# Chyaboiii/antidote_ccrdt

Hardware: AMD Instinct MI355X
Metric: CRDT ops/sec (topk_rmv, 1M keys, 8-DC vclocks) (higher is better)
Workload: dtype int64

## Files before the change

antidote_ccrdt_amd/csrc/engine.cpp:

```cpp
#include <algorithm>
#include <chrono>
#include <cstdio>
#include <cstdlib>
#include <cstring>
#include <mutex>
#include <numeric>
#include <string>
#include <thread>
#include <tuple>
#include <vector>

#include "common.hpp"
#include "engine.hpp"
#include "trmv_kernels.hpp"

namespace ccrdt {

static thread_local std::string g_last_error;
void set_error(const std::string& msg) { g_last_error = msg; }

int trmv_launch_scan(const TrmvApplyArgs& a, uint64_t* partials, uint32_t* key_rmv, hipStream_t st);
void trmv_kernels_preload();
void trmv_wave_preload();
void trmv_resident_preload();
void trmv_steady_preload();
int trmv_launch_validate(const TrmvApplyArgs& a, uint64_t n_ops, uint32_t* err, unsigned long long* scratch,
                         hipStream_t st);
int trmv_launch_mark_done(uint8_t* done, uint64_t n_keys, const uint32_t* list, uint32_t n_list, const uint32_t* n_dev,
                          uint32_t* ex_cnt, hipStream_t st);
int trmv_launch_keep(const TrmvApplyArgs& a, uint32_t grid, hipStream_t st);
int trmv_launch_downstream(const TrmvDownArgs& a, hipStream_t st);
int trmv_launch_wave(const TrmvApplyArgs& a, uint64_t grid_keys, hipStream_t st);
int trmv_launch_first_list(const uint64_t* key_ptr, uint64_t n_keys, uint32_t thresh, uint32_t* list,
                           uint32_t* count, hipStream_t st);
uint32_t trmv_wave_waves(uint64_t grid_keys);
int trmv_launch_resident_consume(const TrmvApplyArgs& a, uint32_t waves, hipStream_t st);
int trmv_launch_steady(const TrmvApplyArgs& a, int cls, uint64_t grid_keys, hipStream_t st);
int trmv_launch_resident(const TrmvApplyArgs& a, uint64_t grid_keys, hipStream_t st);
int trmv_launch_steady_hbm(const TrmvApplyArgs& a, uint32_t waves, void* scratch, hipStream_t st);
uint64_t trmv_steady_hbm_bytes(bool ranked);
uint32_t trmv_steady_hbm_players();
int trmv_launch_replica_vc(const int64_t* vc, uint64_t n_keys, int n_dc, int64_t* out,
                           hipStream_t st);
int trmv_launch_pack_extras(const uint64_t* key_ptr, const uint32_t* ex_cnt, const TrmvExtraRec* ex,
                            const int64_t* ex_vc, uint64_t n_keys, int n_dc, int64_t* rows,
                            int64_t cap, uint32_t* count, hipStream_t st);
int trmv_launch_exchange_pack(const int64_t* vc, const uint64_t* key_ptr, const uint32_t* ex_cnt,
                              const TrmvExtraRec* ex, const int64_t* ex_vc, uint64_t n_keys, int n_dc, int64_t* pack,
                              int64_t cap, const int64_t* op_map, int64_t n_map, uint32_t host_word, hipStream_t st);
int trmv_launch_exchange_reduce(const int64_t* g, int world, int64_t len, int n_dc, int64_t* hdr, int64_t* out,
                                hipStream_t st);

static constexpr int TRMV_N_TIERS = 5;
static constexpr int TRMV_TIER_LAST = 4;
static constexpr uint32_t TRMV_HBM_WAVES = 128;
static constexpr int TRMV_STATUS_WORDS = 2 + 2 * TRMV_N_TIERS;
static constexpr uint32_t TRMV_LATER_GRID = 4096;

template <class F>
void for_key_ranges_host(uint64_t n, F f) {
  const unsigned hw = std::thread::hardware_concurrency();
  uint64_t nt = std::min<uint64_t>(16, hw ? hw : 1);
  nt = std::min<uint64_t>(nt, n / 4096 + 1);
  std::vector<std::thread> pool;
  for (uint64_t t = 1; t < nt; ++t) pool.emplace_back([&, t] { f(n * t / nt, n * (t + 1) / nt); });
  f(0, n / nt);
  for (auto& th : pool) th.join();
}
// ... 319 lines not shown
        used += c - E.arena_sub[0][i][x];
        room += E.arena_sub[1][i][x] - c;
      }
      const uint64_t take = used - std::min(used, E.arena_used[x]);
      E.arena_used[x] = used;
      E.arena_rate[x] = std::max(E.arena_rate[x], take);
      roomy &= room >= 2 * take;
    }
    E.inplace_ready = roomy;
    const uint32_t* lc = reinterpret_cast<const uint32_t*>(static_cast<const char*>(E.h_arena) + 2 * ARENA_RB);
    for (int l = 0; l < 3; ++l) {
      uint32_t n = 0;
      for (int i = 0; i < TRMV_NSUB; ++i) n += lc[4 * i + l];
      E.trmv_overflow_keys[6 + l] = n;
    }
  }
  float mv = 0.f, mr = 0.f;
  CCRDT_HIP(hipEventElapsedTime(&mv, E.evt[0], E.evt[1]));
  CCRDT_HIP(hipEventElapsedTime(&mr, E.evt[1], E.evt[2]));
  E.trmv_tier_ms[5] += mv;
  E.trmv_tier_ms[3] += mr;
  handed = hs[2 + 2 * 3];
  E.trmv_overflow_keys[5] = handed;
  (void)D;
  return CCRDT_OK;
}

int trmv_pass_full(Engine& E, TrmvApplyArgs a, uint64_t n_ops, uint32_t* status, int& first_tier, int& n_over) {
  const int D = E.n_dc;
  const uint64_t nk = (uint64_t)E.n_keys;
  const int out = 1 - E.cur, mout = 1 - E.mcur;
  a.inplace = 0;
  a.fresh = E.fresh ? 1 : 0;
  if (a.key_done) {
    const char* ff = getenv("CCRDT_TRMV_FAIL_FINISH");
    if (ff && ff[0] == '1') {
      set_error("trmv_apply: injected failure of the finishing pass (CCRDT_TRMV_FAIL_FINISH)");
      return CCRDT_ENOMEM;
    }
  }
  a.slack = E.k <= 128 ? trmv_pool_slack() : 0;
  if (E.fresh && !E.fresh_room) a.slack = 0;
  if (E.fresh && a.slack)
    for (int x = 0; x < 3; ++x)
      if (trmv_fresh_off(true, x, nk, n_ops) >= 0xFFFFFFFFull) a.slack = 0;
  a.old_s = E.trmv_side(E.mcur, E.cur);
  CCRDT_TRY(E.trmv[mout].meta.ensure(nk * sizeof(KeyMeta)));
  CCRDT_TRY(E.trmv[mout].cap.ensure(nk * sizeof(KeyCap)));
  a.new_s = E.trmv_side(mout, out);
  const uint64_t nb = (nk + 1023) / 1024;
  CCRDT_TRY(E.partials.ensure((nb * 3 + 3) * sizeof(uint64_t) + nk * sizeof(uint32_t)));
  uint64_t tot[3];
  for (int x = 0; x < 3; ++x) tot[x] = trmv_fresh_off(a.slack != 0, x, nk, n_ops);
  if (!E.fresh && nk) {
    CCRDT_TRY(trmv_launch_scan(a, E.partials.as<uint64_t>(),
                               reinterpret_cast<uint32_t*>(E.partials.as<uint64_t>() + nb * 3 + 3), E.stream));
    CCRDT_HIP(hipMemcpyAsync(E.h_status, E.partials.as<uint64_t>() + nb * 3, 3 * sizeof(uint64_t),
                             hipMemcpyDeviceToHost, E.stream));
    CCRDT_HIP(hipStreamSynchronize(E.stream));
    memcpy(tot, E.h_status, sizeof(tot));
  }
  if (tot[0] >= 0xFFFFFFFFull || tot[1] >= 0xFFFFFFFFull || tot[2] >= 0xFFFFFFFFull) {
    set_error("trmv_apply: resident state would exceed 2^32 elements");
    return CCRDT_ENOMEM;
  }
  auto grow = [&](TrmvBufs& b, bool room) -> int {
// ... 40 lines not shown
  auto segment = [&](int c0, int c1) -> int {
    const int e0 = ev;
    CCRDT_HIP(hipEventRecord(E.evt[ev++], E.stream));
    for (int ci = c0; ci < c1 && nk; ++ci) {
      const int t = chain[ci];
      DevBuf* ovf = &E.tier_ovf[t];
      a.key_list = work ? work->as<uint32_t>() : nullptr;
      a.n_list = work ? 0u : (uint32_t)nk;
      a.n_list_dev = n_dev;
      a.ovf_list = ovf->as<uint32_t>();
      a.status = status + 2 + 2 * t;
      const uint64_t grid = work ? later_grid : nk;
      if (t == 0) CCRDT_TRY(trmv_launch_wave(a, grid, E.stream));
      else if (t == 3) CCRDT_TRY(trmv_launch_resident(a, grid, E.stream));
      else CCRDT_TRY(trmv_launch_steady(a, t - 1, grid, E.stream));
      CCRDT_HIP(hipEventRecord(E.evt[ev++], E.stream));
      work = ovf;
      n_dev = a.status;
    }
    CCRDT_HIP(hipMemcpyAsync(E.h_status, status, TRMV_STATUS_WORDS * 4, hipMemcpyDeviceToHost, E.stream));
    CCRDT_HIP(hipStreamSynchronize(E.stream));
    uint32_t err = 0;
    for (int ci = c0; ci < c1; ++ci) err |= hs[3 + 2 * chain[ci]];
    if (err) return trmv_err_code(err);
    for (int ci = c0; ci < c1 && nk; ++ci) {
      const int t = chain[ci];
      float ms = 0.f;
      CCRDT_HIP(hipEventElapsedTime(&ms, E.evt[e0 + ci - c0], E.evt[e0 + ci - c0 + 1]));
      E.trmv_tier_ms[t] += ms;
      E.trmv_overflow_keys[t] = hs[2 + 2 * t];
    }
    return CCRDT_OK;
  };
  static const bool overlap_env = [] {
    const char* v = getenv("CCRDT_TRMV_OVERLAP");
    return !(v && v[0] == '0');
  }();
  static const uint64_t overlap_keys = [] {
    const char* v = getenv("CCRDT_TRMV_OVERLAP_KEYS");
    return v ? strtoull(v, nullptr, 10) : (1ull << 18);
  }();
  static const uint32_t overlap_waves = [] {
    const char* v = getenv("CCRDT_TRMV_OVERLAP_WAVES");
    const int x = v ? atoi(v) : 32;
    return (uint32_t)(x < 1 ? 1 : (x > 4096 ? 4096 : x));
  }();
  auto head_overlapped = [&]() -> int {
    if (!E.stream2) {
      int lo = 0, hi = 0;
      CCRDT_HIP(hipDeviceGetStreamPriorityRange(&lo, &hi));
      CCRDT_HIP(hipStreamCreateWithPriority(&E.stream2, hipStreamNonBlocking, hi));
      CCRDT_HIP(hipEventCreateWithFlags(&E.ev_ovl, hipEventDisableTiming));
    }
    constexpr uint32_t O_CLAIM = TRMV_NDONE, O_NFIRST = TRMV_NDONE + 1, O_PUB = TRMV_NDONE + 4;
    CCRDT_TRY(E.first_list.ensure(nk * 4));
    CCRDT_TRY(E.ovl.ensure((O_PUB + nk) * 4));
    uint32_t* ov = E.ovl.as<uint32_t>();
    CCRDT_HIP(hipMemsetAsync(ov, 0, (O_PUB + nk) * 4, E.stream));
    const uint32_t pmax = (uint32_t)std::min<int64_t>(E.k, 128);
    const uint32_t thresh = std::min<uint32_t>(128u, pmax + pmax / 5);
    CCRDT_TRY(trmv_launch_first_list(a.key_ptr, nk, thresh, E.first_list.as<uint32_t>(), ov + O_NFIRST, E.stream));
    const int e0 = ev;
    CCRDT_HIP(hipEventRecord(E.evt[ev++], E.stream));
    TrmvApplyArgs a0 = a;
    a0.key_list = nullptr;
    a0.n_list = (uint32_t)nk;
    a0.n_list_dev = nullptr;
    a0.ovf_list = E.tier_ovf[0].as<uint32_t>();
    a0.status = status + 2;
    a0.first_list = E.first_list.as<uint32_t>();
    a0.n_first = ov + O_NFIRST;
    a0.first_thresh = thresh;
    a0.pub = ov + O_PUB;
    a0.n_pub = (uint32_t)nk;
    a0.done = ov;
    CCRDT_TRY(trmv_launch_wave(a0, nk, E.stream));
    CCRDT_HIP(hipEventRecord(E.evt[ev++], E.stream));
    CCRDT_HIP(hipStreamWaitEvent(E.stream2, E.evt[e0], 0));
    TrmvApplyArgs a3 = a;
    a3.key_list = E.tier_ovf[0].as<uint32_t>();
    a3.n_list = 0;
    a3.n_list_dev = status + 2;
    a3.ovf_list = E.tier_ovf[3].as<uint32_t>();
    a3.status = status + 2 + 2 * 3;
    a3.pub = ov + O_PUB;
    a3.n_pub = (uint32_t)nk;
    a3.done = ov;
    a3.prod_waves = trmv_wave_waves(nk);
    a3.claim = ov + O_CLAIM;
    const char* stall_env = getenv("CCRDT_TRMV_OVERLAP_STALL");
    const bool force_stall = stall_env && stall_env[0] == '1';
    a3.spin_limit = force_stall ? 0u : (1u << 19);
    CCRDT_TRY(trmv_launch_resident_consume(a3, overlap_waves, E.stream2));
    CCRDT_HIP(hipEventRecord(E.ev_ovl, E.stream2));
    CCRDT_HIP(hipStreamWaitEvent(E.stream, E.ev_ovl, 0));
    CCRDT_HIP(hipEventRecord(E.evt[ev++], E.stream));
    CCRDT_HIP(hipMemcpyAsync(E.h_status, status, TRMV_STATUS_WORDS * 4, hipMemcpyDeviceToHost, E.stream));
    CCRDT_HIP(hipStreamSynchronize(E.stream));
    if ((hs[3 + 2 * 3] & TRMV_ERR_STALL) || force_stall) {
      CCRDT_HIP(hipMemsetAsync(status + 2 + 2 * 3, 0, 8, E.stream));
      a3.pub = nullptr;
      a3.done = nullptr;
      CCRDT_TRY(trmv_launch_resident(a3, later_grid, E.stream));
      CCRDT_HIP(hipEventRecord(E.evt[ev - 1], E.stream));
      CCRDT_HIP(hipMemcpyAsync(E.h_status, status, TRMV_STATUS_WORDS * 4, hipMemcpyDeviceToHost, E.stream));
      CCRDT_HIP(hipStreamSynchronize(E.stream));
      E.trmv_overflow_keys[9] = 1;
    }
    const uint32_t err = hs[3] | hs[3 + 2 * 3];
    if (err) return trmv_err_code(err);
    float m0 = 0.f, m3 = 0.f;
    CCRDT_HIP(hipEventElapsedTime(&m0, E.evt[e0], E.evt[e0 + 1]));
    CCRDT_HIP(hipEventElapsedTime(&m3, E.evt[e0 + 1], E.evt[e0 + 2]));
    E.trmv_tier_ms[0] += m0;
    E.trmv_tier_ms[3] += m3;
    E.trmv_overflow_keys[0] = hs[2];
    E.trmv_overflow_keys[3] = hs[2 + 2 * 3];
    work = &E.tier_ovf[3];
    n_dev = status + 2 + 2 * 3;
    return CCRDT_OK;
  };
// ... 946 lines not shown
```

antidote_ccrdt_amd/csrc/trmv_kernels.hpp:

```cpp
#pragma once
#include <cstdint>

namespace ccrdt {

constexpr uint32_t NONE16 = 0xFFFFu;
constexpr uint32_t NONE32 = 0xFFFFFFFFu;
constexpr int TRMV_DPAD = 8;
constexpr uint32_t TRMV_SEG_MAX = 0xFFFFu;

struct alignas(32) KeyMeta {
  uint32_t p_off, m_off, r_off;
  uint32_t np;
  uint32_t nm;
  uint32_t nr;
  uint32_t nobs;
  uint32_t minq;
};
static_assert(sizeof(KeyMeta) == 32, "KeyMeta is one 32-byte record");

struct alignas(16) KeyCap {
  uint32_t p_cap, m_cap, r_cap;
  uint16_t m_top;
  uint16_t flags;
};
// ... 37 lines not shown
  const uint8_t* dc;
  const int64_t* ts;
  const int64_t* rmv_vc;
  int64_t n_rmv_rows;
  TrmvSide old_s;
  TrmvSide new_s;
  int32_t fresh;
  uint32_t* ex_cnt;
  TrmvExtraRec* ex;
  int64_t* ex_vc;
  const uint32_t* key_list;
  uint32_t n_list;
  const uint32_t* n_list_dev;
  uint32_t* ovf_list;
  uint32_t* status;
  uint8_t* op_pl;
  int32_t inplace;
  unsigned long long* arena;
  const unsigned long long* arena_lim;
  uint32_t* lay_cnt;
  uint16_t* obs_ord;
  const uint8_t* key_done;
  const uint32_t* verr;
  int32_t slack;
  const uint32_t* first_list;
  const uint32_t* n_first;
  uint32_t first_thresh;
  uint32_t n_pub;
  uint32_t prod_waves;
  uint32_t spin_limit;
  uint32_t* pub;
  uint32_t* done;
  uint32_t* claim;
};
constexpr int TRMV_NDONE = 64;
constexpr uint32_t TRMV_ERR_STALL = 1u << 30;

__device__ __forceinline__ uint32_t trmv_key_nops(const TrmvApplyArgs& a, uint64_t k, uint64_t op0) {
  return (a.key_done && a.key_done[k]) ? 0u : (uint32_t)(a.key_ptr[k + 1] - op0);
}

__device__ __forceinline__ const __attribute__((address_space(4))) TrmvApplyArgs* trmv_kargs() {
  return kernarg_as<TrmvApplyArgs>();
}

__host__ __device__ __forceinline__ uint64_t trmv_fresh_off(bool room, int x, uint64_t k, uint64_t o) {
  return room ? (x == 0 ? 3 * o + 16 * k : (x == 1 ? 6 * o + 32 * k : o + 8 * k)) : o;
}
__host__ __device__ __forceinline__ uint32_t trmv_fresh_cap(bool room, int x, uint32_t nops) {
  return room ? (x == 0 ? 3 * nops + 16 : (x == 1 ? 6 * nops + 32 : nops + 8)) : nops;
}

__device__ __forceinline__ KeyMeta trmv_new_meta(const TrmvApplyArgs& a, uint64_t k) {
  if (a.fresh) {
    KeyMeta m;
    const uint64_t o = a.key_ptr[k];
    m.p_off = (uint32_t)trmv_fresh_off(a.slack != 0, 0, k, o);
    m.m_off = (uint32_t)trmv_fresh_off(a.slack != 0, 1, k, o);
    m.r_off = (uint32_t)trmv_fresh_off(a.slack != 0, 2, k, o);
    m.np = m.nm = m.nr = m.nobs = 0;
    m.minq = NONE32;
    return m;
  }
  return a.new_s.meta[k];
}

// ... 26 lines not shown
```

antidote_ccrdt_amd/csrc/trmv_wave.hip:

```cpp
#include "common.hpp"
#include "trmv_kernels.hpp"

#ifdef TRMV_PROF
__device__ unsigned long long g_trmv_prof[16];
#define PROF_STAMP(v)                                                        \
  do {                                                                       \
    __builtin_amdgcn_sched_barrier(0);                                       \
    asm volatile("s_memtime %0\n\ts_waitcnt lgkmcnt(0)" : "=s"(v)::"memory"); \
    __builtin_amdgcn_sched_barrier(0);                                       \
  } while (0)
#define PROF_MARK(i)                                                         \
  do {                                                                       \
    unsigned long long _t;                                                   \
    PROF_STAMP(_t);                                                          \
    if (lane_id() == 0 && (key & 63u) == 3) atomicAdd(&g_trmv_prof[i], _t - prof_t);             \
    prof_t = _t;                                                             \
  } while (0)
#else
#define PROF_STAMP(v) (void)0
#define PROF_MARK(i) (void)0
#endif

namespace ccrdt {

namespace {
constexpr int W_HCAP = 256;
constexpr int W_ECAP = 128;
constexpr int W_PCAP = 128;
constexpr int W_RCAP = 24;
constexpr int W_WAVES = 1;
#define ST_OUT(p, v) (*(p) = (v))
#define LD_IN(p) (*(p))
constexpr int W_KPW = 8;
constexpr int W_MD = (W_KPW + 7) / 8;
static_assert(W_KPW >= 1 && W_KPW <= 64, "1..64 keys per wave chunk");
constexpr unsigned long long W_EMPTY = 0x8000000000000000ull;
constexpr uint32_t NONE8 = 0xFFu;
constexpr uint32_t HSINK = W_HCAP, ESINK = W_ECAP, PSINK = W_PCAP;

template <bool FRESH>
struct alignas(16) WaveLds {
  static constexpr int NS_ = FRESH ? 0 : 1;
  unsigned long long htab[W_HCAP + 2];
  int64_t esc[W_ECAP + 2];
  int64_t ets[W_ECAP + 2];
  int64_t rows[W_RCAP][TRMV_DPAD];
  unsigned long long vc[TRMV_DPAD + 2];
  uint32_t pcnt2[W_PCAP / 2 + 4];
  uint32_t rsrc[W_RCAP];
  uint16_t ekd[W_ECAP + 8];
  uint8_t hp[W_HCAP];
  uint8_t sorted[W_ECAP + 8];
  uint8_t slab[W_ECAP];
  uint8_t fin[NS_ * (W_ECAP + 8)];
  uint32_t pa[W_PCAP + 8];
  uint32_t pb[W_PCAP + 8];
  uint8_t pmoff[NS_ * (W_PCAP + 8)];
  uint8_t peb[NS_ * (W_PCAP + 8)];
  uint8_t cpl[W_PCAP + 8];
  uint8_t rl[W_RCAP + 8];
  uint32_t nex;
  __device__ __forceinline__ uint8_t& fa(uint32_t p, int b) { return reinterpret_cast<uint8_t*>(pa)[4 * p + b]; }
  __device__ __forceinline__ uint8_t& fb(uint32_t p, int b) { return reinterpret_cast<uint8_t*>(pb)[4 * p + b]; }
};
#define PSTART(p) L.fa((p), 0)
#define PLR(p) L.fa((p), 1)
#define PFLAG(p) L.fa((p), 2)
#define PCNTF(p) L.fa((p), 3)
#define POBS(p) L.fb((p), 0)
#define PROW(p) L.fb((p), 1)
#define PGB(p) L.fb((p), 2)
#define PSLOT(p) L.fb((p), 3)

#define KA trmv_kargs()

__device__ __forceinline__ uint32_t whash(int64_t id) {
  const uint64_t x = (uint64_t)id * 0x9E3779B97F4A7C15ull;
  return (uint32_t)(x >> 56);
}

template <class W>
__device__ __forceinline__ uint32_t pcnt_of(const W& L, uint32_t p) {
  return (L.pcnt2[p >> 1] >> (16 * (p & 1))) & 0xFFFFu;
}

template <class W>
__device__ __forceinline__ void wave_emit(const TrmvApplyArgs& a, W& L, uint64_t op0,
                                          uint64_t op, uint8_t kind, int64_t id, int64_t sc,
                                          uint32_t dc, int64_t ts, uint32_t row) {
  const uint32_t pos = atomicAdd(&L.nex, 1u);
  TrmvExtraRec r;
  r.op = (uint32_t)op;
  r.kind = kind;
  r.dc = (uint8_t)dc;
  r.pad = 0;
  r.id = id;
  r.score = sc;
  r.ts = ts;
  KA->ex[op0 + pos] = r;
  if (kind == CCRDT_TRMV_RMV)
    for (int d = 0; d < KA->n_dc; ++d) KA->ex_vc[(op0 + pos) * KA->n_dc + d] = L.rows[row][d];
}

struct KeyIn {
  uint64_t op0;
  uint32_t nops;
  KeyMeta nmeta;
  int64_t id[2], sc[2], ts[2];
  uint32_t kind[2], dc[2];
  int64_t rv[W_RCAP / 8];
};

struct ChunkHdr {
  uint32_t key;
  uint64_t lo, hi;
  uint32_t meta[W_MD];
  uint64_t skip;
};

__device__ __forceinline__ uint32_t wave_list_key(uint32_t i, uint32_t n_first) {
  if (KA->first_list) return i < n_first ? KA->first_list[i] : i - n_first;
  return KA->key_list ? KA->key_list[i] : i;
}

__device__ __forceinline__ void wave_load_chunk(const TrmvApplyArgs& a, uint32_t c0, uint32_t n,
                                                uint32_t n_first, ChunkHdr& h) {
  const int lane = lane_id();
  const uint32_t j = (uint32_t)lane < n ? (uint32_t)lane : 0u;
  h.key = wave_list_key(c0 + j, n_first);
  h.lo = KA->key_ptr[h.key];
  h.hi = KA->key_ptr[h.key + 1];
  h.skip = KA->first_list ? ballot((uint32_t)lane < n && c0 + j >= n_first && h.hi - h.lo > KA->first_thresh) : 0ull;
#pragma unroll
  for (int i = 0; i < W_MD; ++i) {
    const uint32_t m = 8 * i + (lane >> 3);
    const uint32_t jm = m < n ? m : 0u;
    const uint32_t km = shfl32(h.key, (int)jm);
    if (KA->fresh) {
      const uint32_t d = lane & 7;
      h.meta[i] = d < 3 ? (uint32_t)trmv_fresh_off(KA->slack != 0, (int)d, km, KA->key_ptr[km])
                        : (d == 7 ? NONE32 : 0u);
    } else {
      h.meta[i] = reinterpret_cast<const uint32_t*>(a.new_s.meta + km)[lane & 7];
    }
  }
}

__device__ __forceinline__ void wave_load_key(const TrmvApplyArgs& a, const ChunkHdr& h, uint32_t j,
                                              KeyIn& in) {
  const int lane = lane_id();
  in.op0 = (uint64_t)rl64((int64_t)h.lo, (int)j);
  in.nops = (uint32_t)((uint64_t)rl64((int64_t)h.hi, (int)j) - in.op0);
  uint32_t* m = reinterpret_cast<uint32_t*>(&in.nmeta);
#pragma unroll
  for (int d = 0; d < 8; ++d) {
    uint32_t v = 0;
#pragma unroll
    for (int i = 0; i < W_MD; ++i)
      if ((j >> 3) == (uint32_t)i) v = rl32(h.meta[i], (int)(8 * (j & 7) + d));
    m[d] = v;
  }
  const int64_t* idp = KA->id + in.op0;
  const int64_t* scp = KA->score + in.op0;
  const int64_t* tsp = KA->ts + in.op0;
  const uint8_t* kp = KA->kind + in.op0;
  const uint8_t* dp = KA->dc + in.op0;
#pragma unroll
  for (int s = 0; s < 2; ++s) {
    const uint32_t l = s * 64 + lane;
    const bool v = l < in.nops;
    in.id[s] = v ? LD_IN(idp + l) : 0;
    in.sc[s] = v ? LD_IN(scp + l) : 0;
    in.ts[s] = v ? LD_IN(tsp + l) : 0;
    in.kind[s] = v ? (uint32_t)LD_IN(kp + l) : 0u;
    in.dc[s] = v ? (uint32_t)LD_IN(dp + l) : 0u;
  }
}

template <class W>
__device__ __forceinline__ void wave_load_rows(const TrmvApplyArgs& a, W& L, KeyIn& in) {
  const int lane = lane_id();
#pragma unroll
  for (int s = 0; s < W_RCAP / 8; ++s) in.rv[s] = 0;
  bool r[2];
#pragma unroll
  for (int s = 0; s < 2; ++s)
    r[s] = (uint32_t)(s * 64 + lane) < in.nops && (in.kind[s] == 2 || in.kind[s] == 3);
  const uint64_t b0 = ballot(r[0]), b1 = ballot(r[1]);
  const uint32_t n0 = (uint32_t)__builtin_popcountll(b0);
  const uint32_t n = n0 + (uint32_t)__builtin_popcountll(b1);
  if (n == 0 || KA->n_rmv_rows <= 0) return;
#pragma unroll
  for (int s = 0; s < 2; ++s) {
    const uint32_t k = s ? n0 + mbcnt(b1) : mbcnt(b0);
    if (r[s] && k < (uint32_t)W_RCAP)
      L.rsrc[k] = (in.ts[s] >= 0 && in.ts[s] < KA->n_rmv_rows) ? (uint32_t)in.ts[s] : 0u;
  }
  wave_lds_sync();
  const uint32_t d = (lane & 7) < KA->n_dc ? (lane & 7) : 0u;
#pragma unroll
  for (int s = 0; s < W_RCAP / 8; ++s) {
    const uint32_t k = s * 8 + (lane >> 3);
    const uint32_t row = k < n ? L.rsrc[k] : 0u;
    in.rv[s] = KA->rmv_vc[(uint64_t)row * KA->n_dc + d];
  }
  wave_lds_sync();
}

enum : int { W_DONE = 0, W_NEXT_TIER = 1, W_REJECT = 2 };

template <bool FRESH>
__device__ __forceinline__ int trmv_wave_key(const TrmvApplyArgs& a, uint32_t key, const KeyIn& in,
                                              WaveLds<FRESH>& L, bool has_next, const ChunkHdr& hdr,
                                              uint32_t nj, KeyIn& nxt) {
  int lane = lane_id();
  asm volatile("" : "+v"(lane));
  const int D = KA->n_dc;
#ifdef TRMV_PROF
  unsigned long long prof_t;
  PROF_STAMP(prof_t);
#endif
  const uint64_t op0 = in.op0;
  const uint32_t nops = in.nops;
  KeyMeta nmeta = in.nmeta;
  nmeta.p_off = __builtin_amdgcn_readfirstlane(nmeta.p_off);
  nmeta.m_off = __builtin_amdgcn_readfirstlane(nmeta.m_off);
  nmeta.r_off = __builtin_amdgcn_readfirstlane(nmeta.r_off);
  KeyMeta om;
  if (FRESH) {
    om.p_off = om.m_off = om.r_off = 0;
    om.np = om.nm = om.nr = om.nobs = 0;
    om.minq = NONE32;
  } else {
    om = a.old_s.meta[key];
  }
  const uint32_t pmax = KA->k < (uint32_t)W_PCAP ? KA->k : (uint32_t)W_PCAP;
  if (nops > (uint32_t)W_ECAP || om.np > pmax || om.nm + nops > (uint32_t)W_ECAP ||
      om.nr > (uint32_t)W_RCAP)
    return W_NEXT_TIER;

  int64_t xsc[2] = {in.sc[0], in.sc[1]};
  const int64_t xts[2] = {in.ts[0], in.ts[1]};
  const uint32_t xkind[2] = {in.kind[0], in.kind[1]};
  const uint32_t xdc[2] = {in.dc[0], in.dc[1]};
  const bool xv[2] = {(uint32_t)lane < nops, (uint32_t)(64 + lane) < nops};
  int64_t pid[2] = {0, 0};
  uint32_t pinfo[2] = {NONE32, NONE32}, pslab[2] = {0u, 0u};
// ... 119 lines not shown
        PSLOT(p) = (uint8_t)hs[2 + s];
        bad |= ((pslab[s] >> 16) != 0) != ((pinfo[s] & 0xFFFFu) != NONE16);
      }
    }
    if (ballot(bad)) return W_NEXT_TIER;
  }
  wave_lds_sync();
  uint32_t np;
  {
    const unsigned long long* h4 = &L.htab[lane * 4];
    const unsigned long long t0 = h4[0], t1 = h4[1], t2 = h4[2], t3 = h4[3];
    const uint32_t hp4 = reinterpret_cast<const uint32_t*>(L.hp)[lane];
    const uint32_t n0 = (t0 != W_EMPTY && (hp4 & 0xFFu) == NONE8) ? 1u : 0u;
    const uint32_t n1 = (t1 != W_EMPTY && ((hp4 >> 8) & 0xFFu) == NONE8) ? 1u : 0u;
    const uint32_t n2 = (t2 != W_EMPTY && ((hp4 >> 16) & 0xFFu) == NONE8) ? 1u : 0u;
    const uint32_t n3 = (t3 != W_EMPTY && (hp4 >> 24) == NONE8) ? 1u : 0u;
    const uint32_t c = n0 + n1 + n2 + n3;
    const uint64_t b0 = ballot(c & 1), b1 = ballot(c & 2), b2 = ballot(c & 4);
    const uint32_t base = om.np + mbcnt(b0) + 2 * mbcnt(b1) + 4 * mbcnt(b2);
    np = om.np + (uint32_t)__builtin_popcountll(b0) + 2 * (uint32_t)__builtin_popcountll(b1) +
         4 * (uint32_t)__builtin_popcountll(b2);
    if (np > pmax) return W_NEXT_TIER;
    const uint32_t i0 = base, i1 = i0 + n0, i2 = i1 + n1, i3 = i2 + n2;
    const uint32_t nhp = (n0 ? i0 : (hp4 & 0xFFu)) | ((n1 ? i1 : ((hp4 >> 8) & 0xFFu)) << 8) |
                         ((n2 ? i2 : ((hp4 >> 16) & 0xFFu)) << 16) |
                         ((n3 ? i3 : (hp4 >> 24)) << 24);
    reinterpret_cast<uint32_t*>(L.hp)[lane] = nhp;
    if (n0) PSLOT(i0) = (uint8_t)(lane * 4 + 0);
    if (n1) PSLOT(i1) = (uint8_t)(lane * 4 + 1);
    if (n2) PSLOT(i2) = (uint8_t)(lane * 4 + 2);
    if (n3) PSLOT(i3) = (uint8_t)(lane * 4 + 3);
  }
  wave_lds_sync();
  if (FRESH && has_next) wave_load_key(a, hdr, nj, nxt);

  PROF_MARK(2);
  uint32_t xrank[2], xp[2];
  {
    uint32_t hpv[2], cr[2];
#pragma unroll
    for (int s = 0; s < 2; ++s) hpv[s] = L.hp[hs[s]];
#pragma unroll
    for (int s = 0; s < 2; ++s) {
      const uint32_t p = xv[s] ? hpv[s] : PSINK;
      xp[s] = p;
      if (xa[s]) atomicMax(&L.vc[xdc[s]], (unsigned long long)xts[s]);
      if (!FRESH && xr[s]) PFLAG(p) = 1;
      cr[s] = atomicAdd(&L.pcnt2[(xv[s] ? p : (uint32_t)lane) >> 1], xv[s] ? 1u << (16 * (p & 1)) : 0u);
    }
#pragma unroll
    for (int s = 0; s < 2; ++s) xrank[s] = xv[s] ? (cr[s] >> (16 * (xp[s] & 1))) & 0xFFFFu : 0u;
  }
  wave_lds_sync();
  {
    uint32_t tot0, tot1;
    const uint32_t c0 = (uint32_t)lane < np ? pcnt_of(L, lane) : 0u;
    const uint32_t c1 = (uint32_t)(64 + lane) < np ? pcnt_of(L, 64 + lane) : 0u;
    const uint32_t st0 = wave_excl_scan_dpp(c0, tot0);
    const uint32_t st1 = wave_excl_scan_dpp(c1, tot1);
    PSTART(lane) = (uint8_t)st0;
    PSTART(64 + lane) = (uint8_t)(tot0 + st1);
  }
  wave_lds_sync();
  uint32_t xq[2], xst[2], xc[2];
#pragma unroll
  for (int s = 0; s < 2; ++s) {
    xst[s] = PSTART(xp[s]);
// ... 40 lines not shown
      wave_lds_sync();
#pragma unroll
      for (int s = 0; s < 2; ++s)
        if (xv[s])
          for (uint32_t x = 0; x < xc[s]; ++x)
            if (L.sorted[xst[s] + x] == (uint32_t)(s * 64 + lane)) xq[s] = xst[s] + x;
    }
  }
  if (!FRESH) {
    uint32_t ebase = nops;
#pragma unroll
    for (int s = 0; s < 2; ++s) {
      const uint32_t p = s * 64 + lane;
      const uint32_t oc = p < om.np ? (pslab[s] >> 16) : 0u;
      uint32_t tot;
      const uint32_t eb = ebase + wave_excl_scan_dpp(oc, tot);
      ebase += tot;
      if (p < om.np) {
        L.peb[p] = (uint8_t)eb;
        PFLAG(p) = 1;
      }
      for (uint32_t j = 0; j < oc; ++j) {
        const uint32_t go = (pslab[s] & 0xFFFFu) + j;
        const uint32_t e = eb + j;
        L.esc[e] = (a.old_s.m_score + om.m_off)[go];
        L.ets[e] = (a.old_s.m_ts + om.m_off)[go];
        L.ekd[e] = (uint16_t)(((uint32_t)(a.old_s.m_dc + om.m_off)[go] << 2) | (p << 8));
      }
    }
  }
  wave_lds_sync();

  PROF_MARK(3);
  if (!FRESH && has_next) wave_load_key(a, hdr, nj, nxt);
  if (!FRESH) {
    bool simple[2], beaten[2] = {false, false}, gbeaten[2] = {false, false}, risk[2] = {false, false};
    uint32_t me[2], cl[2];
#pragma unroll
    for (int s = 0; s < 2; ++s) {
      simple[s] = xa[s] && !PFLAG(xp[s]);
      me[s] = xq[s] - xst[s];
      cl[s] = simple[s] ? xc[s] : 0u;
    }
    const uint32_t maxc = wave_max_u32_dpp(cl[0] > cl[1] ? cl[0] : cl[1]);
    for (uint32_t x = 0; x < maxc; ++x) {
#pragma unroll
      for (int s = 0; s < 2; ++s) {
        const bool valid = x < cl[s] && x != me[s];
        const uint32_t pos = x < cl[s] ? xst[s] + x : (uint32_t)ESINK;
        const int64_t sx = L.esc[pos], tx = L.ets[pos];
        const uint32_t dx = (L.ekd[pos] >> 2) & 7u;
        const int64_t sm = xsc[s], tm = xts[s];
        const bool before = x < me[s];
        risk[s] |= valid && before && tx >= tm;
        beaten[s] |= valid && (sx > sm || (sx == sm && (before ? tx >= tm : tx > tm)));
        gbeaten[s] |= valid && (sx > sm || (sx == sm && (dx > xdc[s] || (dx == xdc[s] && tx > tm))));
      }
    }
#pragma unroll
    for (int s = 0; s < 2; ++s) {
      if (risk[s]) PFLAG(xp[s]) = 1;
      if (simple[s] && !beaten[s]) POBS(xp[s]) = (uint8_t)xq[s];
      if (simple[s] && !gbeaten[s]) PGB(xp[s]) = (uint8_t)xq[s];
    }
    wave_lds_sync();
  } else {
    uint8_t* const cq = L.slab;
// ... 71 lines not shown
      if (act) mrg[k] = (uint8_t)(yr && !first);
      any_merge |= ballot(yr && !first) != 0;
    }
    wave_lds_sync();
    if (any_merge) {
#pragma unroll 1
      for (uint32_t b = 0; b < mn; b += 64) {
        const uint32_t k = b + lane;
        const uint32_t q = k < mn && mrg[k] ? (uint32_t)cq[k] : ESINK;
        const uint32_t p = q != ESINK ? (uint32_t)(L.ekd[q] >> 8) : PSINK;
        if (q != ESINK && !PFLAG(p)) {
          unsigned long long* dst = reinterpret_cast<unsigned long long*>(L.rows[PROW(p)]);
          const int64_t* src = L.rows[(uint32_t)L.esc[q]];
          for (int d = 0; d < D; ++d) atomicMax(dst + d, (unsigned long long)src[d]);
        }
      }
    }
    wave_lds_sync();
  }

  PROF_MARK(6);
  uint32_t ncx;
  {
    const bool c0 = (uint32_t)lane < np && PFLAG(lane);
    const bool c1 = (uint32_t)(64 + lane) < np && PFLAG(64 + lane);
    const uint64_t m0 = ballot(c0), m1 = ballot(c1);
    const uint32_t n0 = (uint32_t)__builtin_popcountll(m0);
    ncx = n0 + (uint32_t)__builtin_popcountll(m1);
    if (c0) L.cpl[mbcnt(m0)] = (uint8_t)lane;
    if (c1) L.cpl[n0 + mbcnt(m1)] = (uint8_t)(64 + lane);
  }
  wave_lds_sync();
  __builtin_amdgcn_s_waitcnt(0x0F70);
  if (FRESH && has_next) wave_load_rows(a, L, nxt);
  PROF_MARK(7);
  uint32_t best_q = NONE32;
  int64_t best_sc = INT64_MAX, best_id = INT64_MAX;
  auto min_cand = [&](bool has, int64_t sc, int64_t id, uint32_t p) {
    const bool better = has && (best_q == NONE32 || sc < best_sc || (sc == best_sc && id < best_id));
    best_q = better ? p : best_q;
    best_sc = better ? sc : best_sc;
    best_id = better ? id : best_id;
  };
  if (FRESH) {
#pragma unroll
    for (int s = 0; s < 2; ++s) {
      const uint32_t q = s * 64 + lane;
      const uint32_t qq = q < nops ? q : (uint32_t)ESINK;
      const int64_t sc = L.esc[qq], ts = L.ets[qq];
      const uint32_t kd = L.ekd[qq];
      if (q < nops) {
        ST_OUT((KA->new_s.m_score + nmeta.m_off) + (q), sc);
        ST_OUT((KA->new_s.m_ts + nmeta.m_off) + (q), ts);
        ST_OUT((KA->new_s.m_dc + nmeta.m_off) + (q), (uint8_t)((kd >> 2) & 7u));
      }
    }
  }
  uint32_t mbase = 0;
#pragma unroll 1
  for (uint32_t b = 0; b < ncx; b += 64) {
    const uint32_t k = b + lane;
    const bool act = k < ncx;
    const uint32_t p = act ? L.cpl[k] : 0u;
    uint32_t ocnt = 0, pinfo_p = NONE32, eb = 0;
    if (!FRESH && act && p < om.np) {
      pinfo_p = (a.old_s.pl_info + om.p_off)[p];
// ... 94 lines not shown
        }
      }
    }
    if (FRESH) {
      uint32_t opos = NONE16, gj = 0;
      for (uint32_t j = 0; j < cnt; ++j) {
        const uint32_t e2 = L.slab[moff + j];
        const int64_t s2 = L.esc[e2], t2 = L.ets[e2];
        const uint32_t d2 = (L.ekd[e2] >> 2) & 7u;
        ST_OUT((KA->new_s.m_score + nmeta.m_off) + (st + j), s2);
        ST_OUT((KA->new_s.m_ts + nmeta.m_off) + (st + j), t2);
        ST_OUT((KA->new_s.m_dc + nmeta.m_off) + (st + j), (uint8_t)d2);
        opos = e2 == o ? j : opos;
        const uint32_t eb = L.slab[moff + gj];
        const int64_t bs = L.esc[eb], bt = L.ets[eb];
        const uint32_t bd = (L.ekd[eb] >> 2) & 7u;
        if (s2 > bs || (s2 == bs && (d2 > bd || (d2 == bd && t2 > bt)))) gj = j;
      }
      if (act) {
        POBS(p) = (uint8_t)(o == NONE8 ? NONE8 : st + opos);
        PGB(p) = (uint8_t)(st + gj);
        PCNTF(p) = (uint8_t)cnt;
        PROW(p) = (uint8_t)prow;
      }
      min_cand(act && o != NONE8, osc, id, p);
    } else if (act) {
      POBS(p) = (uint8_t)o;
      PCNTF(p) = (uint8_t)cnt;
      L.pmoff[p] = (uint8_t)moff;
      PROW(p) = (uint8_t)prow;
    }
  }
  wave_lds_sync();
  if (!FRESH && has_next) wave_load_rows(a, L, nxt);

  PROF_MARK(4);
  uint32_t fbase = 0, rbase = 0, nobs = 0;
  uint32_t po[2] = {NONE8, NONE8};
  if (FRESH) {
    uint32_t csum = 0;
#pragma unroll
    for (int s = 0; s < 2; ++s) {
      const uint32_t p = s * 64 + lane;
      const bool act = p < np;
      const uint32_t pp = act ? p : (uint32_t)PSINK;
      const uint32_t wa = L.pa[pp], wb = L.pb[pp];
      const uint32_t st = wa & 0xFFu, c = pcnt_of(L, pp), lrp = (wa >> 8) & 0xFFu;
      const bool replayed = ((wa >> 16) & 0xFFu) != 0;
      const uint32_t off = (replayed || lrp == 0) ? st : lrp;
      const uint32_t cnt = act ? (replayed ? (wa >> 24) : st + c - off) : 0u;
      const uint32_t o = act ? (wb & 0xFFu) : NONE8;
      const uint32_t prow = act ? ((wb >> 8) & 0xFFu) : NONE8;
      const uint64_t rm = ballot(prow != NONE8);
      const uint32_t rix = rbase + mbcnt(rm);
      rbase += (uint32_t)__builtin_popcountll(rm);
      if (prow != NONE8) L.rl[rix] = (uint8_t)prow;
      const int64_t id = (int64_t)L.htab[wb >> 24];
      const uint32_t gb = (replayed || cnt > 1) ? ((wb >> 16) & 0xFFu) - off : 0u;
      if (act) {
        ST_OUT((KA->new_s.pl_id + nmeta.p_off) + (p), id);
        ST_OUT((KA->new_s.pl_slab + nmeta.p_off) + (p), off | (cnt << 16));
        if (cnt > 1) ST_OUT((KA->new_s.pl_gb + nmeta.p_off) + (p), (uint16_t)gb);
        ST_OUT(KA->new_s.pl_info + nmeta.p_off + p, (o == NONE8 ? NONE16 : o - off) |
                                             ((prow != NONE8 ? rix : NONE16) << 16));
      }
      csum += cnt;
// ... 117 lines not shown
      const uint64_t hit = ballot(has && best_sc == ms && best_id == mi);
      best_q = rl32(best_q, (int)__builtin_ctzll(hit));
    }
  }
  if (lane == 0) {
    KeyMeta out = nmeta;
    out.np = np;
    out.nm = fbase;
    out.nr = rbase;
    out.nobs = nobs;
    out.minq = best_q;
    KA->new_s.meta[key] = out;
    KA->ex_cnt[key] = L.nex;
    if (FRESH && KA->slack) {
      KeyCap c;
      c.p_cap = trmv_fresh_cap(true, 0, nops);
      c.m_cap = trmv_fresh_cap(true, 1, nops);
      c.r_cap = trmv_fresh_cap(true, 2, nops);
      c.m_top = (uint16_t)nops;
      c.flags = TRMV_CAP_VALID;
      KA->new_s.cap[key] = c;
    }
  }
  PROF_MARK(5);
  return W_DONE;
}
}

template <bool FRESH, int OCC>
__global__ __launch_bounds__(64 * W_WAVES, OCC) void trmv_wave_kernel(TrmvApplyArgs a) {
  __shared__ WaveLds<FRESH> lds[W_WAVES];
  const uint32_t wv = __builtin_amdgcn_readfirstlane(threadIdx.x >> 6);
  WaveLds<FRESH>& L = lds[wv];
  const uint32_t n_first = a.first_list ? *a.n_first : 0u;
  const uint32_t n = (a.n_list_dev ? *a.n_list_dev : a.n_list) + n_first;
  for (uint32_t c0 = (blockIdx.x * W_WAVES + wv) * W_KPW; c0 < n; c0 += gridDim.x * W_WAVES * W_KPW) {
    const uint32_t cn = c0 + W_KPW < n ? W_KPW : n - c0;
    ChunkHdr hdr;
    wave_load_chunk(a, c0, cn, n_first, hdr);
    KeyIn cur, nxt;
    wave_load_key(a, hdr, 0, cur);
    __builtin_amdgcn_s_waitcnt(0x0F70);
    wave_load_rows(a, L, cur);
    for (uint32_t j = 0; j < cn; ++j) {
      const uint32_t key = rl32(hdr.key, (int)j);
      const bool has_next = j + 1 < cn;
      const int r = (hdr.skip >> j) & 1u ? W_REJECT + 1
                                         : trmv_wave_key<FRESH>(a, key, cur, L, has_next, hdr, j + 1, nxt);
      if (r != W_DONE) {
        if (r == W_NEXT_TIER && lane_id() == 0) {
          const uint32_t pos = atomicAdd(&KA->status[0], 1u);
          KA->ovf_list[pos] = key;
          if (KA->pub && pos < KA->n_pub) {
            const uint32_t old = atomicExch(&KA->pub[pos], key + 1u);
            __builtin_amdgcn_s_waitcnt(0x0F70);
            asm volatile("" ::"v"(old));
          }
        }
        if (has_next) wave_load_key(a, hdr, j + 1, nxt);
        __builtin_amdgcn_s_waitcnt(0x0F70);
        if (has_next) wave_load_rows(a, L, nxt);
      }
      wave_lds_sync();
      cur = nxt;
    }
  }
  if (a.done && lane_id() == 0) atomicAdd(&KA->done[(blockIdx.x * W_WAVES + wv) % TRMV_NDONE], 1u);
}

void trmv_wave_preload() {
  preload_kernels(trmv_wave_kernel<true, 5>, trmv_wave_kernel<false, 5>, trmv_wave_kernel<true, 4>);
}

uint32_t trmv_wave_waves(uint64_t grid_keys) {
  const uint64_t per_block = (uint64_t)W_WAVES * W_KPW;
  return (uint32_t)((grid_keys + per_block - 1) / per_block) * W_WAVES;
}

int trmv_launch_wave(const TrmvApplyArgs& a, uint64_t grid_keys, hipStream_t st) {
  if (grid_keys == 0) return CCRDT_OK;
  const uint64_t per_block = (uint64_t)W_WAVES * W_KPW;
  const uint64_t blocks = (grid_keys + per_block - 1) / per_block;
  if (a.fresh)
    if (a.pub)
      hipLaunchKernelGGL((trmv_wave_kernel<true, 4>), dim3((unsigned)blocks), dim3(64 * W_WAVES), 0, st, a);
    else
      hipLaunchKernelGGL((trmv_wave_kernel<true, 5>), dim3((unsigned)blocks), dim3(64 * W_WAVES), 0, st, a);
  else
    hipLaunchKernelGGL((trmv_wave_kernel<false, 5>), dim3((unsigned)blocks), dim3(64 * W_WAVES), 0, st, a);
  CCRDT_HIP(hipGetLastError());
  return CCRDT_OK;
}

}

#ifdef TRMV_PROF
extern "C" int ccrdt_debug_trmv_prof(unsigned long long* out16, int reset) {
  if (hipMemcpyFromSymbol(out16, HIP_SYMBOL(g_trmv_prof), 16 * 8) != hipSuccess) return 4;
  if (reset) {
    unsigned long long z[16] = {};
    if (hipMemcpyToSymbol(HIP_SYMBOL(g_trmv_prof), z, sizeof(z)) != hipSuccess) return 4;
  }
  return 0;
}
#endif
```

Before: 46.59 billion.

## Prefetch next chunk headers and add dynamic chunk claiming to wave kernel

Reworks the wave kernel's chunk loop. Per-key bounds and metadata are now loaded lazily per key rather than all up front per chunk. The next chunk's key_ptr header is staged through LDS while the current key is still being processed, and the next chunk index is claimed through an atomic counter (wave_claim) rather than a fixed grid stride. An optional block-count cap, sized from occupancy, is added but disabled by default. The aim is to hide header-load latency across chunk boundaries and balance uneven per-key work, at the cost of an atomic per chunk, more LDS syncs, and reusing the hp buffer for rsrc.

```diff
diff --git a/antidote_ccrdt_amd/csrc/engine.cpp b/antidote_ccrdt_amd/csrc/engine.cpp
--- a/antidote_ccrdt_amd/csrc/engine.cpp
+++ b/antidote_ccrdt_amd/csrc/engine.cpp
@@ -33,7 +33,7 @@
 int trmv_launch_wave(const TrmvApplyArgs& a, uint64_t grid_keys, hipStream_t st);
 int trmv_launch_first_list(const uint64_t* key_ptr, uint64_t n_keys, uint32_t thresh, uint32_t* list,
                            uint32_t* count, hipStream_t st);
-uint32_t trmv_wave_waves(uint64_t grid_keys);
+uint32_t trmv_wave_waves(const TrmvApplyArgs& a, uint64_t grid_keys);
 int trmv_launch_resident_consume(const TrmvApplyArgs& a, uint32_t waves, hipStream_t st);
 int trmv_launch_steady(const TrmvApplyArgs& a, int cls, uint64_t grid_keys, hipStream_t st);
 int trmv_launch_resident(const TrmvApplyArgs& a, uint64_t grid_keys, hipStream_t st);
@@ -419,6 +419,7 @@
   const int out = 1 - E.cur, mout = 1 - E.mcur;
   a.inplace = 0;
   a.fresh = E.fresh ? 1 : 0;
+  a.wave_claim = status;
   if (a.key_done) {
     const char* ff = getenv("CCRDT_TRMV_FAIL_FINISH");
     if (ff && ff[0] == '1') {
@@ -525,7 +526,7 @@
     }
     return CCRDT_OK;
   };
-  static const bool overlap_env = [] {
+  const bool overlap_env = [] {
     const char* v = getenv("CCRDT_TRMV_OVERLAP");
     return !(v && v[0] == '0');
   }();
@@ -579,7 +580,7 @@
     a3.pub = ov + O_PUB;
     a3.n_pub = (uint32_t)nk;
     a3.done = ov;
-    a3.prod_waves = trmv_wave_waves(nk);
+    a3.prod_waves = trmv_wave_waves(a0, nk);
     a3.claim = ov + O_CLAIM;
     const char* stall_env = getenv("CCRDT_TRMV_OVERLAP_STALL");
     const bool force_stall = stall_env && stall_env[0] == '1';
diff --git a/antidote_ccrdt_amd/csrc/trmv_kernels.hpp b/antidote_ccrdt_amd/csrc/trmv_kernels.hpp
--- a/antidote_ccrdt_amd/csrc/trmv_kernels.hpp
+++ b/antidote_ccrdt_amd/csrc/trmv_kernels.hpp
@@ -93,6 +93,7 @@
   uint32_t* pub;
   uint32_t* done;
   uint32_t* claim;
+  uint32_t* wave_claim;
 };
 constexpr int TRMV_NDONE = 64;
 constexpr uint32_t TRMV_ERR_STALL = 1u << 30;
diff --git a/antidote_ccrdt_amd/csrc/trmv_wave.hip b/antidote_ccrdt_amd/csrc/trmv_wave.hip
--- a/antidote_ccrdt_amd/csrc/trmv_wave.hip
+++ b/antidote_ccrdt_amd/csrc/trmv_wave.hip
@@ -32,8 +32,7 @@
 #define ST_OUT(p, v) (*(p) = (v))
 #define LD_IN(p) (*(p))
 constexpr int W_KPW = 8;
-constexpr int W_MD = (W_KPW + 7) / 8;
-static_assert(W_KPW >= 1 && W_KPW <= 64, "1..64 keys per wave chunk");
+static_assert(W_KPW >= 2 && W_KPW <= 63, "2..63 keys per wave chunk");
 constexpr unsigned long long W_EMPTY = 0x8000000000000000ull;
 constexpr uint32_t NONE8 = 0xFFu;
 constexpr uint32_t HSINK = W_HCAP, ESINK = W_ECAP, PSINK = W_PCAP;
@@ -47,7 +46,7 @@
   int64_t rows[W_RCAP][TRMV_DPAD];
   unsigned long long vc[TRMV_DPAD + 2];
   uint32_t pcnt2[W_PCAP / 2 + 4];
-  uint32_t rsrc[W_RCAP];
+  uint32_t nkp[W_KPW + 1];
   uint16_t ekd[W_ECAP + 8];
   uint8_t hp[W_HCAP];
   uint8_t sorted[W_ECAP + 8];
@@ -113,53 +112,69 @@
 
 struct ChunkHdr {
   uint32_t key;
-  uint64_t lo, hi;
-  uint32_t meta[W_MD];
-  uint64_t skip;
+  uint32_t lo, hi;
 };
-
-__device__ __forceinline__ uint32_t wave_list_key(uint32_t i, uint32_t n_first) {
-  if (KA->first_list) return i < n_first ? KA->first_list[i] : i - n_first;
-  return KA->key_list ? KA->key_list[i] : i;
-}
-
-__device__ __forceinline__ void wave_load_chunk(const TrmvApplyArgs& a, uint32_t c0, uint32_t n,
-                                                uint32_t n_first, ChunkHdr& h) {
+__device__ __forceinline__ uint32_t wave_key_ptr(uint32_t k) {
+  return reinterpret_cast<const uint32_t*>(KA->key_ptr)[2 * (uint64_t)k];
+}
+
+__device__ __forceinline__ void wave_load_hdr(uint32_t c0, uint32_t n, uint32_t n_first, ChunkHdr& h) {
+  const uint32_t l = (uint32_t)lane_id() < n ? (uint32_t)lane_id() : 0u;
+  const uint32_t i = c0 + l;
+  if (KA->first_list) h.key = i < n_first ? KA->first_list[i] : i - n_first;
+  else h.key = KA->key_list ? KA->key_list[i] : i;
+  h.lo = wave_key_ptr(h.key);
+  h.hi = wave_key_ptr(h.key + 1);
+}
+
+__device__ __forceinline__ uint32_t wave_lane_here() {
+  uint32_t lane = (uint32_t)lane_id();
+  asm volatile("" : "+v"(lane));
+  return lane;
+}
+__device__ __forceinline__ bool wave_hdr_stageable(uint32_t c1, uint32_t n_first) {
+  return !KA->key_list && c1 >= n_first;
+}
+__device__ __forceinline__ uint32_t wave_stage_hdr(uint32_t c1, uint32_t n1, uint32_t n_first) {
+  const uint32_t lane = wave_lane_here();
+  const uint32_t l = lane <= n1 ? lane : 0u;
+  return wave_key_ptr(c1 - n_first + l);
+}
+template <class W>
+__device__ __forceinline__ void wave_commit_hdr(W& L, uint32_t stg) {
+  const uint32_t lane = wave_lane_here();
+  if (lane <= (uint32_t)W_KPW) L.nkp[lane] = stg;
+  wave_lds_sync();
+}
+template <class W>
+__device__ __forceinline__ void wave_take_hdr(W& L, uint32_t c1, uint32_t n_first, ChunkHdr& h) {
+  wave_lds_sync();
+  const uint32_t lane = wave_lane_here();
+  const uint32_t l = lane < (uint32_t)W_KPW ? lane : 0u;
+  h.key = c1 - n_first + l;
+  h.lo = L.nkp[l];
+  h.hi = L.nkp[l + 1];
+}
+
+template <bool FRESH>
+__device__ __forceinline__ void wave_key_bounds(const TrmvApplyArgs& a, const ChunkHdr& h, uint32_t hl,
+                                                KeyIn& in) {
+  in.op0 = (uint64_t)rl32(h.lo, (int)hl);
+  in.nops = rl32(h.hi, (int)hl) - (uint32_t)in.op0;
+  const uint32_t key = rl32(h.key, (int)hl);
+  if (FRESH) {
+    in.nmeta.p_off = (uint32_t)trmv_fresh_off(KA->slack != 0, 0, key, in.op0);
+    in.nmeta.m_off = (uint32_t)trmv_fresh_off(KA->slack != 0, 1, key, in.op0);
+    in.nmeta.r_off = (uint32_t)trmv_fresh_off(KA->slack != 0, 2, key, in.op0);
+    in.nmeta.np = in.nmeta.nm = in.nmeta.nr = in.nmeta.nobs = 0;
+    in.nmeta.minq = NONE32;
+  } else {
+    in.nmeta = KA->new_s.meta[key];
+  }
+}
+
+__device__ __forceinline__ void wave_load_ops(const TrmvApplyArgs& a, KeyIn& in) {
   const int lane = lane_id();
-  const uint32_t j = (uint32_t)lane < n ? (uint32_t)lane : 0u;
-  h.key = wave_list_key(c0 + j, n_first);
-  h.lo = KA->key_ptr[h.key];
-  h.hi = KA->key_ptr[h.key + 1];
-  h.skip = KA->first_list ? ballot((uint32_t)lane < n && c0 + j >= n_first && h.hi - h.lo > KA->first_thresh) : 0ull;
-#pragma unroll
-  for (int i = 0; i < W_MD; ++i) {
-    const uint32_t m = 8 * i + (lane >> 3);
-    const uint32_t jm = m < n ? m : 0u;
-    const uint32_t km = shfl32(h.key, (int)jm);
-    if (KA->fresh) {
-      const uint32_t d = lane & 7;
-      h.meta[i] = d < 3 ? (uint32_t)trmv_fresh_off(KA->slack != 0, (int)d, km, KA->key_ptr[km])
-                        : (d == 7 ? NONE32 : 0u);
-    } else {
-      h.meta[i] = reinterpret_cast<const uint32_t*>(a.new_s.meta + km)[lane & 7];
-    }
-  }
-}
-
-__device__ __forceinline__ void wave_load_key(const TrmvApplyArgs& a, const ChunkHdr& h, uint32_t j,
-                                              KeyIn& in) {
-  const int lane = lane_id();
-  in.op0 = (uint64_t)rl64((int64_t)h.lo, (int)j);
-  in.nops = (uint32_t)((uint64_t)rl64((int64_t)h.hi, (int)j) - in.op0);
-  uint32_t* m = reinterpret_cast<uint32_t*>(&in.nmeta);
-#pragma unroll
-  for (int d = 0; d < 8; ++d) {
-    uint32_t v = 0;
-#pragma unroll
-    for (int i = 0; i < W_MD; ++i)
-      if ((j >> 3) == (uint32_t)i) v = rl32(h.meta[i], (int)(8 * (j & 7) + d));
-    m[d] = v;
-  }
   const int64_t* idp = KA->id + in.op0;
   const int64_t* scp = KA->score + in.op0;
   const int64_t* tsp = KA->ts + in.op0;
@@ -190,29 +205,59 @@
   const uint32_t n0 = (uint32_t)__builtin_popcountll(b0);
   const uint32_t n = n0 + (uint32_t)__builtin_popcountll(b1);
   if (n == 0 || KA->n_rmv_rows <= 0) return;
+  static_assert(W_HCAP >= 4 * W_RCAP, "hp holds the staged rows");
+  uint32_t* const rsrc = reinterpret_cast<uint32_t*>(L.hp);
 #pragma unroll
   for (int s = 0; s < 2; ++s) {
     const uint32_t k = s ? n0 + mbcnt(b1) : mbcnt(b0);
     if (r[s] && k < (uint32_t)W_RCAP)
-      L.rsrc[k] = (in.ts[s] >= 0 && in.ts[s] < KA->n_rmv_rows) ? (uint32_t)in.ts[s] : 0u;
+      rsrc[k] = (in.ts[s] >= 0 && in.ts[s] < KA->n_rmv_rows) ? (uint32_t)in.ts[s] : 0u;
   }
   wave_lds_sync();
   const uint32_t d = (lane & 7) < KA->n_dc ? (lane & 7) : 0u;
 #pragma unroll
   for (int s = 0; s < W_RCAP / 8; ++s) {
     const uint32_t k = s * 8 + (lane >> 3);
-    const uint32_t row = k < n ? L.rsrc[k] : 0u;
+    const uint32_t row = k < n ? rsrc[k] : 0u;
     in.rv[s] = KA->rmv_vc[(uint64_t)row * KA->n_dc + d];
   }
   wave_lds_sync();
 }
 
 enum : int { W_DONE = 0, W_NEXT_TIER = 1, W_REJECT = 2 };
+
+struct WaveNext {
+  bool has_next;
+  uint32_t nl;
+  bool stage;
+  bool take;
+  bool staged;
+  uint32_t c1, n1;
+  uint32_t n_first;
+  bool claim;
+};
+
+template <bool FRESH>
+__device__ __forceinline__ void wave_issue_next(const TrmvApplyArgs& a, WaveLds<FRESH>& L, ChunkHdr& hdr,
+                                                const WaveNext& nx, KeyIn& nxt, uint32_t& stg, uint32_t& clm) {
+  if (nx.claim) {
+    uint32_t* const cp = KA->wave_claim;
+    if (wave_lane_here() == 0) clm = atomicAdd(cp, 1u);
+  }
+  if (nx.take) {
+    if (nx.staged) wave_take_hdr(L, nx.c1, nx.n_first, hdr);
+    else wave_load_hdr(nx.c1, nx.n1, nx.n_first, hdr);
+  }
+  if (nx.has_next) wave_key_bounds<FRESH>(a, hdr, nx.nl, nxt);
+  if (nx.stage) stg = wave_stage_hdr(nx.c1, nx.n1, nx.n_first);
+  if (nx.has_next) wave_load_ops(a, nxt);
+}
 
 template <bool FRESH>
 __device__ __forceinline__ int trmv_wave_key(const TrmvApplyArgs& a, uint32_t key, const KeyIn& in,
-                                              WaveLds<FRESH>& L, bool has_next, const ChunkHdr& hdr,
-                                              uint32_t nj, KeyIn& nxt) {
+                                              WaveLds<FRESH>& L, ChunkHdr& hdr, const WaveNext& nx,
+                                              KeyIn& nxt, uint32_t& clm) {
+  const bool has_next = nx.has_next;
   int lane = lane_id();
   asm volatile("" : "+v"(lane));
   const int D = KA->n_dc;
@@ -398,7 +443,8 @@
     if (n3) PSLOT(i3) = (uint8_t)(lane * 4 + 3);
   }
   wave_lds_sync();
-  if (FRESH && has_next) wave_load_key(a, hdr, nj, nxt);
+  uint32_t stg = 0;
+  if (FRESH) wave_issue_next<FRESH>(a, L, hdr, nx, nxt, stg, clm);
 
   PROF_MARK(2);
   uint32_t xrank[2], xp[2];
@@ -505,7 +551,7 @@
   wave_lds_sync();
 
   PROF_MARK(3);
-  if (!FRESH && has_next) wave_load_key(a, hdr, nj, nxt);
+  if (!FRESH) wave_issue_next<FRESH>(a, L, hdr, nx, nxt, stg, clm);
   if (!FRESH) {
     bool simple[2], beaten[2] = {false, false}, gbeaten[2] = {false, false}, risk[2] = {false, false};
     uint32_t me[2], cl[2];
@@ -643,6 +689,8 @@
   }
   wave_lds_sync();
   __builtin_amdgcn_s_waitcnt(0x0F70);
+  clm = __builtin_amdgcn_readfirstlane(clm);
+  if (FRESH && nx.stage) wave_commit_hdr(L, stg);
   if (FRESH && has_next) wave_load_rows(a, L, nxt);
   PROF_MARK(7);
   uint32_t best_q = NONE32;
@@ -803,6 +851,8 @@
     }
   }
   wave_lds_sync();
+  if (!FRESH) clm = __builtin_amdgcn_readfirstlane(clm);
+  if (!FRESH && nx.stage) wave_commit_hdr(L, stg);
   if (!FRESH && has_next) wave_load_rows(a, L, nxt);
 
   PROF_MARK(4);
@@ -986,62 +1036,124 @@
   __shared__ WaveLds<FRESH> lds[W_WAVES];
   const uint32_t wv = __builtin_amdgcn_readfirstlane(threadIdx.x >> 6);
   WaveLds<FRESH>& L = lds[wv];
-  const uint32_t n_first = a.first_list ? *a.n_first : 0u;
-  const uint32_t n = (a.n_list_dev ? *a.n_list_dev : a.n_list) + n_first;
-  for (uint32_t c0 = (blockIdx.x * W_WAVES + wv) * W_KPW; c0 < n; c0 += gridDim.x * W_WAVES * W_KPW) {
-    const uint32_t cn = c0 + W_KPW < n ? W_KPW : n - c0;
+  WaveNext nx;
+  nx.n_first = a.first_list ? *a.n_first : 0u;
+  const uint32_t n = (a.n_list_dev ? *a.n_list_dev : a.n_list) + nx.n_first;
+  const uint32_t waves = gridDim.x * W_WAVES;
+  uint32_t c0 = (blockIdx.x * W_WAVES + wv) * W_KPW;
+  uint32_t c1 = c0 + waves * W_KPW, c2 = 0;
+  if (c0 < n) {
+    uint32_t cn = c0 + W_KPW < n ? W_KPW : n - c0;
     ChunkHdr hdr;
-    wave_load_chunk(a, c0, cn, n_first, hdr);
+    wave_load_hdr(c0, cn, nx.n_first, hdr);
     KeyIn cur, nxt;
-    wave_load_key(a, hdr, 0, cur);
+    wave_key_bounds<FRESH>(a, hdr, 0, cur);
+    wave_load_ops(a, cur);
     __builtin_amdgcn_s_waitcnt(0x0F70);
     wave_load_rows(a, L, cur);
-    for (uint32_t j = 0; j < cn; ++j) {
-      const uint32_t key = rl32(hdr.key, (int)j);
-      const bool has_next = j + 1 < cn;
-      const int r = (hdr.skip >> j) & 1u ? W_REJECT + 1
-                                         : trmv_wave_key<FRESH>(a, key, cur, L, has_next, hdr, j + 1, nxt);
-      if (r != W_DONE) {
-        if (r == W_NEXT_TIER && lane_id() == 0) {
-          const uint32_t pos = atomicAdd(&KA->status[0], 1u);
-          KA->ovf_list[pos] = key;
-          if (KA->pub && pos < KA->n_pub) {
-            const uint32_t old = atomicExch(&KA->pub[pos], key + 1u);
-            __builtin_amdgcn_s_waitcnt(0x0F70);
-            asm volatile("" ::"v"(old));
+    for (;;) {
+      nx.c1 = c1;
+      const bool more = c1 > c0 && c1 < n;
+      nx.n1 = more ? (nx.c1 + W_KPW < n ? W_KPW : n - nx.c1) : 0u;
+      nx.staged = more && wave_hdr_stageable(nx.c1, nx.n_first);
+      for (uint32_t j = 0; j < cn; ++j) {
+        const uint32_t key = rl32(hdr.key, (int)j);
+        const bool last = j + 1 == cn;
+        nx.has_next = !last || more;
+        nx.nl = last ? 0u : j + 1;
+        nx.stage = nx.staged && j == 0;
+        nx.take = more && last;
+        nx.claim = more && j == 0;
+        uint32_t clm = 0;
+        const bool skip = a.first_list && c0 + j >= nx.n_first && cur.nops > a.first_thresh;
+        const int r = skip ? W_REJECT + 1 : trmv_wave_key<FRESH>(a, key, cur, L, hdr, nx, nxt, clm);
+        if (r != W_DONE) {
+          if (r == W_NEXT_TIER && lane_id() == 0) {
+            const uint32_t pos = atomicAdd(&KA->status[0], 1u);
+            KA->ovf_list[pos] = key;
+            if (KA->pub && pos < KA->n_pub) {
+              const uint32_t old = atomicExch(&KA->pub[pos], key + 1u);
+              __builtin_amdgcn_s_waitcnt(0x0F70);
+              asm volatile("" ::"v"(old));
+            }
           }
+          uint32_t stg = 0;
+          wave_issue_next<FRESH>(a, L, hdr, nx, nxt, stg, clm);
+          __builtin_amdgcn_s_waitcnt(0x0F70);
+          if (nx.stage) wave_commit_hdr(L, stg);
+          if (nx.has_next) wave_load_rows(a, L, nxt);
+          clm = __builtin_amdgcn_readfirstlane(clm);
         }
-        if (has_next) wave_load_key(a, hdr, j + 1, nxt);
-        __builtin_amdgcn_s_waitcnt(0x0F70);
-        if (has_next) wave_load_rows(a, L, nxt);
-      }
-      wave_lds_sync();
-      cur = nxt;
+        if (nx.claim) c2 = (2 * waves + clm) * W_KPW;
+        wave_lds_sync();
+        cur = nxt;
+      }
+      if (!more) break;
+      c0 = c1;
+      c1 = c2;
+      cn = nx.n1;
     }
   }
   if (a.done && lane_id() == 0) atomicAdd(&KA->done[(blockIdx.x * W_WAVES + wv) % TRMV_NDONE], 1u);
+}
+
+namespace {
+constexpr int W_MAXDEV = 64;
+constexpr bool W_PERSIST = false;
+uint32_t g_wave_fill[W_MAXDEV][3];
+uint32_t g_wave_cap;
+
+int wave_inst(const TrmvApplyArgs& a) { return a.fresh ? (a.pub ? 2 : 0) : 1; }
+
+uint32_t wave_blocks(int inst, uint64_t grid_keys) {
+  const uint64_t per_block = (uint64_t)W_WAVES * W_KPW;
+  uint64_t blocks = (grid_keys + per_block - 1) / per_block;
+  int dev = 0;
+  if (hipGetDevice(&dev) != hipSuccess || dev < 0 || dev >= W_MAXDEV) dev = 0;
+  const uint32_t fill = g_wave_cap ? g_wave_cap : (W_PERSIST && inst != 2 ? g_wave_fill[dev][inst] : 0u);
+  if (fill) blocks = std::min<uint64_t>(blocks, fill);
+  return (uint32_t)blocks;
+}
 }
 
 void trmv_wave_preload() {
   preload_kernels(trmv_wave_kernel<true, 5>, trmv_wave_kernel<false, 5>, trmv_wave_kernel<true, 4>);
-}
-
-uint32_t trmv_wave_waves(uint64_t grid_keys) {
-  const uint64_t per_block = (uint64_t)W_WAVES * W_KPW;
-  return (uint32_t)((grid_keys + per_block - 1) / per_block) * W_WAVES;
+  const char* v = getenv("CCRDT_TRMV_WAVE_BLOCKS");
+  const long cap = v ? atol(v) : 0;
+  g_wave_cap = cap > 0 ? (uint32_t)std::min<long>(cap, 1l << 30) : 0u;
+  int dev = 0, cus = 0;
+  if (hipGetDevice(&dev) != hipSuccess || dev < 0 || dev >= W_MAXDEV) return;
+  if (hipDeviceGetAttribute(&cus, hipDeviceAttributeMultiprocessorCount, dev) != hipSuccess || cus <= 0) {
+    (void)hipGetLastError();
+    return;
+  }
+  const void* kern[3] = {reinterpret_cast<const void*>(trmv_wave_kernel<true, 5>),
+                         reinterpret_cast<const void*>(trmv_wave_kernel<false, 5>),
+                         reinterpret_cast<const void*>(trmv_wave_kernel<true, 4>)};
+  for (int i = 0; i < 3; ++i) {
+    int per_cu = 0;
+    if (hipOccupancyMaxActiveBlocksPerMultiprocessor(&per_cu, kern[i], 64 * W_WAVES, 0) != hipSuccess || per_cu <= 0) {
+      (void)hipGetLastError();
+      continue;
+    }
+    g_wave_fill[dev][i] = (uint32_t)per_cu * (uint32_t)cus;
+  }
+}
+
+uint32_t trmv_wave_waves(const TrmvApplyArgs& a, uint64_t grid_keys) {
+  return wave_blocks(wave_inst(a), grid_keys) * W_WAVES;
 }
 
 int trmv_launch_wave(const TrmvApplyArgs& a, uint64_t grid_keys, hipStream_t st) {
   if (grid_keys == 0) return CCRDT_OK;
-  const uint64_t per_block = (uint64_t)W_WAVES * W_KPW;
-  const uint64_t blocks = (grid_keys + per_block - 1) / per_block;
-  if (a.fresh)
-    if (a.pub)
-      hipLaunchKernelGGL((trmv_wave_kernel<true, 4>), dim3((unsigned)blocks), dim3(64 * W_WAVES), 0, st, a);
-    else
-      hipLaunchKernelGGL((trmv_wave_kernel<true, 5>), dim3((unsigned)blocks), dim3(64 * W_WAVES), 0, st, a);
+  const int inst = wave_inst(a);
+  const uint32_t blocks = wave_blocks(inst, grid_keys);
+  if (inst == 2)
+    hipLaunchKernelGGL((trmv_wave_kernel<true, 4>), dim3(blocks), dim3(64 * W_WAVES), 0, st, a);
+  else if (inst == 0)
+    hipLaunchKernelGGL((trmv_wave_kernel<true, 5>), dim3(blocks), dim3(64 * W_WAVES), 0, st, a);
   else
-    hipLaunchKernelGGL((trmv_wave_kernel<false, 5>), dim3((unsigned)blocks), dim3(64 * W_WAVES), 0, st, a);
+    hipLaunchKernelGGL((trmv_wave_kernel<false, 5>), dim3(blocks), dim3(64 * W_WAVES), 0, st, a);
   CCRDT_HIP(hipGetLastError());
   return CCRDT_OK;
 }
```

Result: faster. 47.16 billion, median of 6 (+1.2%).
